# nanoporetech/medaka

Measured on NVIDIA H100. Metric: pileup positions/sec (consensus inference), higher is better.
Workload: dtype f32

## Files before the change

### medaka_b200/csrc/gru_wg.cu

```cuda
#include "common.cuh"
#include "ptx.cuh"
#include "rec_common.cuh"

namespace mdk {

constexpr int RW_THREADS = 256;
constexpr int RW_ABLK = (H / 8) * 64 * 16;
constexpr int RW_XBLK = 2 * 64 * 16;

template <int NT, bool FUSE_X, int OUT>
struct RwCfg {
    static constexpr int N = NT * RT_N;
    static constexpr bool HL = NT == 1;
    static constexpr int ROWS = HL ? 2 * N : N;
    static constexpr int PLANES = HL ? 1 : 2;
    static constexpr int KG = ROWS * 16 + 16;
    static constexpr int HPLANE = (H / 8) * KG;
    static constexpr int XPLANE = 2 * KG;
    static constexpr int HLO = HL ? N * 16 : HPLANE;
    static constexpr int XLO = HL ? N * 16 : XPLANE;
    static constexpr int RED = (RW_THREADS / 32) * NCLS * N;
    static constexpr int wlo_off = 0;
    static constexpr int wxlo_off = wlo_off + 6 * RW_ABLK;
    static constexpr int h_off = wxlo_off + (FUSE_X ? 6 * RW_XBLK : 0);
// ... 331 lines not shown
    dim3 grid((unsigned)((tiles + NT - 1) / NT), NDIR);
    constexpr bool LOGITS = OUT == OUT_LOGITS;
    kern<<<grid, RW_THREADS, smem_bytes, s>>>(gi, xin, w_hh_tm, b_hn, LOGITS ? nullptr : out, B, T, lin_w,
                                              LOGITS ? static_cast<float *>(out) : nullptr);
    return cudaGetLastError();
}

template <int NT>
static cudaError_t launch_rec_nt(const float *gi, const RecX *xin, const __half *w_hh_tm, const float *b_hn, int out_kind,
                                 void *out, const float *lin_w, int64_t B, int64_t T, cudaStream_t s) {
    if (xin)
        return out_kind == OUT_TILES ? launch_rec<NT, true, OUT_TILES>(gi, *xin, w_hh_tm, b_hn, out, nullptr, B, T, s)
                                     : cudaErrorInvalidValue;
    const RecX none{nullptr, nullptr, nullptr, 0};
    switch (out_kind) {
    case OUT_TILES: return launch_rec<NT, false, OUT_TILES>(gi, none, w_hh_tm, b_hn, out, nullptr, B, T, s);
    case OUT_ROWS: return launch_rec<NT, false, OUT_ROWS>(gi, none, w_hh_tm, b_hn, out, nullptr, B, T, s);
    case OUT_LOGITS:
        return lin_w ? launch_rec<NT, false, OUT_LOGITS>(gi, none, w_hh_tm, b_hn, out, lin_w, B, T, s) : cudaErrorInvalidValue;
    }
    return cudaErrorInvalidValue;
}

cudaError_t launch_rec_tc(const float *gi, const RecX *xin, const __half *w_hh_tm, const float *b_hn, int tiles_per_cta,
                          int out_kind, void *out, const float *lin_w, int64_t B, int64_t T, cudaStream_t s) {
    if (B == 0 || T == 0) return cudaSuccess;
    switch (tiles_per_cta) {
    case 1: return launch_rec_nt<1>(gi, xin, w_hh_tm, b_hn, out_kind, out, lin_w, B, T, s);
    case 2: return launch_rec_nt<2>(gi, xin, w_hh_tm, b_hn, out_kind, out, lin_w, B, T, s);
    }
    return cudaErrorInvalidValue;
}

constexpr int GW_THREADS = 256;
constexpr int GW_QK = 8;
constexpr int GW_STAGE_PLANE = GW_QK * XT_ROWS * 16;
constexpr int GW_STAGE = 2 * GW_STAGE_PLANE;
constexpr int GW_NQ = XT_K / 8 / GW_QK;
constexpr int GW_X_OFF = XT_TILE_BYTES;
constexpr int GW_BAR_OFF = GW_X_OFF + 2 * GW_STAGE;
constexpr int GW_SMEM = GW_BAR_OFF + 16;

__global__ void __launch_bounds__(GW_THREADS, 1)
gemm_tc_kernel(const uint8_t *__restrict__ x_tiles, const __half *__restrict__ w_in_tm, const float *__restrict__ bias,
               float *__restrict__ gi, int64_t P, int64_t ntiles) {
    extern __shared__ __align__(128) uint8_t smem[];
    uint64_t *full = reinterpret_cast<uint64_t *>(smem + GW_BAR_OFF);
    const int tid = threadIdx.x, wg = tid >> 7, warp = (tid >> 5) & 3, lane = tid & 31;
    const int gq = lane >> 2, cq = lane & 3;
    const int blk = blockIdx.x;
    const uint32_t sbase = smem_u32(smem);
    for (int i = tid; i < 2 * H * (H2 / 8); i += GW_THREADS) {
        const int kg = i & 31, r = (i >> 5) & (H - 1), p = i >> 12;
        const uint4 v = reinterpret_cast<const uint4 *>(w_in_tm + (((size_t)blk * 2 + p) * H + r) * H2)[kg];
        *reinterpret_cast<uint4 *>(smem + p * XT_PLANE_BYTES + kg * (XT_ROWS * 16) + r * 16) = v;
    }
    if (tid == 0) {
        mbar_init(&full[0], 1);
        mbar_init(&full[1], 1);
        fence_mbar_init();
    }
    fence_proxy_async_smem();
    __syncthreads();
    const int64_t my_tiles = blockIdx.y < ntiles ? (ntiles - 1 - blockIdx.y) / gridDim.y + 1 : 0;
    const int64_t nst = my_tiles * GW_NQ;
    auto issue = [&](int64_t it) {
        const int64_t tile = blockIdx.y + (it / GW_NQ) * gridDim.y;
        const int q = (int)(it % GW_NQ), s = (int)(it & 1);
        const uint8_t *src = x_tiles + tile * (int64_t)XT_TILE_BYTES + q * GW_STAGE_PLANE;
        mbar_arrive_expect_tx(&full[s], GW_STAGE);
        bulk_g2s(smem + GW_X_OFF + s * GW_STAGE, src, GW_STAGE_PLANE, &full[s]);
        bulk_g2s(smem + GW_X_OFF + s * GW_STAGE + GW_STAGE_PLANE, src + XT_PLANE_BYTES, GW_STAGE_PLANE, &full[s]);
    };
    if (tid == 0) {
        if (nst > 0) issue(0);
        if (nst > 1) issue(1);
    }
    const float bj[2] = {bias[blk * H + wg * 64 + warp * 16 + gq], bias[blk * H + wg * 64 + warp * 16 + gq + 8]};
    float acc[64];
#pragma unroll 1
    for (int64_t it = 0; it < nst; ++it) {
        const int q = (int)(it % GW_NQ), s = (int)(it & 1);
        mbar_wait(&full[s], (uint32_t)((it >> 1) & 1));
        wg_fence();
#pragma unroll
        for (int prod = 0; prod < 3; ++prod) {
            const int pa = prod == 2, pb = prod == 1;
#pragma unroll
            for (int kk = 0; kk < GW_QK / 2; ++kk) {
                const uint64_t a = make_smem_desc(sbase + pa * XT_PLANE_BYTES + (q * GW_QK + 2 * kk) * (XT_ROWS * 16) + wg * 64 * 16,
                                                  XT_ROWS * 16, 128);
                const uint64_t b = make_smem_desc(sbase + GW_X_OFF + s * GW_STAGE + pb * GW_STAGE_PLANE + 2 * kk * (XT_ROWS * 16),
                                                  XT_ROWS * 16, 128);
                Wgmma<128>::ss(acc, a, b, (q | prod | kk) ? 1u : 0u);
            }
        }
        wg_commit();
        wg_wait_all();
        wg_hold(acc);
        __syncthreads();
        if (tid == 0 && it + 2 < nst) issue(it + 2);
        if (q == GW_NQ - 1) {
            const int64_t tile = blockIdx.y + (it / GW_NQ) * gridDim.y;
            const int64_t prem = P - tile * XT_ROWS;
#pragma unroll
            for (int k = 0; k < 64; k += 2) {
                const int c = 8 * (k >> 2) + 2 * cq, hb = (k >> 1) & 1;
                if (c >= prem) continue;
                const int j = wg * 64 + warp * 16 + gq + 8 * hb;
                float *o = gi + ((((tile * (XT_ROWS / WT) + (c >> 4)) * 6 + blk) * 4 + ((c & 15) >> 2)) * H + j) * 4 + (c & 3);
                __stcs(reinterpret_cast<float2 *>(o), make_float2(acc[k] + bj[hb], acc[k + 1] + bj[hb]));
            }
        }
    }
}

cudaError_t launch_gemm_tc(const void *x_tiles, const __half *w_in_tm, const float *bias, float *gi, int64_t P,
                           int sm_count, cudaStream_t s) {
    if (P == 0) return cudaSuccess;
    const int64_t ntiles = (P + XT_ROWS - 1) / XT_ROWS;
    cudaError_t ea = cudaFuncSetAttribute(gemm_tc_kernel, cudaFuncAttributeMaxDynamicSharedMemorySize, GW_SMEM);
    if (ea != cudaSuccess) return ea;
    int64_t ct = sm_count / 6;
    if (ct < 1) ct = 1;
    if (ct > ntiles) ct = ntiles;
    dim3 grid(6, (unsigned)ct);
    gemm_tc_kernel<<<grid, GW_THREADS, GW_SMEM, s>>>(reinterpret_cast<const uint8_t *>(x_tiles), w_in_tm, bias, gi, P, ntiles);
    return cudaGetLastError();
}

__global__ void __launch_bounds__(256, 1)
selftest_kernel(const float *__restrict__ A, const float *__restrict__ Bm, float *__restrict__ D, int N, int K) {
    extern __shared__ __align__(128) uint8_t smem[];
    const int a_plane = 128 * K * 2, b_plane = N * K * 2;
    uint8_t *sa = smem, *sb = smem + 2 * a_plane;
    const int tid = threadIdx.x, wg = tid >> 7, warp = (tid >> 5) & 3, lane = tid & 31;
    for (int i = tid; i < 128 * K; i += 256) {
        const int r = i / K, k = i % K;
        __half hi, lo;
        split_f16(A[i], hi, lo);
        const int off = (k / 8) * (128 * 16) + r * 16 + (k % 8) * 2;
        *reinterpret_cast<__half *>(sa + off) = hi;
        *reinterpret_cast<__half *>(sa + a_plane + off) = lo;
    }
    for (int i = tid; i < N * K; i += 256) {
        const int r = i / K, k = i % K;
        __half hi, lo;
        split_f16(Bm[i], hi, lo);
        const int off = (k / 8) * (N * 16) + r * 16 + (k % 8) * 2;
        *reinterpret_cast<__half *>(sb + off) = hi;
        *reinterpret_cast<__half *>(sb + b_plane + off) = lo;
    }
    fence_proxy_async_smem();
    __syncthreads();
    for (int n0 = 0; n0 < N; n0 += 16) {
        float d[8];
        wg_fence();
        uint32_t acc = 0;
        for (int prod = 0; prod < 3; ++prod) {
            const int pa = (prod == 2), pb = (prod == 1);
// ... 40 lines not shown
```

### medaka_b200/csrc/ptx.cuh

```cuda
#pragma once
#include <cstdint>
#include <cuda_fp16.h>

namespace mdk {

__device__ __forceinline__ uint32_t smem_u32(const void *p) {
    return static_cast<uint32_t>(__cvta_generic_to_shared(p));
}

__device__ __forceinline__ void mbar_init(uint64_t *bar, uint32_t count) {
    asm volatile("mbarrier.init.shared::cta.b64 [%0], %1;" ::"r"(smem_u32(bar)), "r"(count) : "memory");
}
__device__ __forceinline__ void fence_mbar_init() {
    asm volatile("fence.mbarrier_init.release.cluster;" ::: "memory");
}
__device__ __forceinline__ void mbar_arrive_expect_tx(uint64_t *bar, uint32_t bytes) {
    asm volatile("mbarrier.arrive.expect_tx.shared::cta.b64 _, [%0], %1;" ::"r"(smem_u32(bar)), "r"(bytes)
                 : "memory");
}
__device__ __forceinline__ bool mbar_try_wait(uint64_t *bar, uint32_t parity) {
    uint32_t ok;
    asm volatile(
        "{\n\t.reg .pred p;\n\t"
        "mbarrier.try_wait.parity.shared::cta.b64 p, [%1], %2;\n\t"
        "selp.u32 %0, 1, 0, p;\n\t}"
        : "=r"(ok)
        : "r"(smem_u32(bar)), "r"(parity)
        : "memory");
    return ok != 0;
}
__device__ __forceinline__ void mbar_wait(uint64_t *bar, uint32_t parity) {
    if (mbar_try_wait(bar, parity)) return;
    const long long t0 = clock64();
    while (!mbar_try_wait(bar, parity)) {
        if (clock64() - t0 > 4000000000LL) __trap();
    }
}

__device__ __forceinline__ void fence_proxy_async_smem() {
    asm volatile("fence.proxy.async.shared::cta;" ::: "memory");
}

__device__ __forceinline__ uint32_t cluster_ctarank() {
    uint32_t r;
    asm volatile("mov.u32 %0, %%cluster_ctarank;" : "=r"(r));
    return r;
}
__device__ __forceinline__ uint32_t mapa_shared(uint32_t smem_addr, uint32_t rank) {
    uint32_t r;
    asm volatile("mapa.shared::cluster.u32 %0, %1, %2;" : "=r"(r) : "r"(smem_addr), "r"(rank));
    return r;
// ... 1 lines not shown
__device__ __forceinline__ void st_cluster_u32(uint32_t cluster_addr, uint32_t v) {
    asm volatile("st.shared::cluster.u32 [%0], %1;" ::"r"(cluster_addr), "r"(v) : "memory");
}
__device__ __forceinline__ void fence_proxy_async_cluster() {
    asm volatile("fence.proxy.async.shared::cluster;" ::: "memory");
}
__device__ __forceinline__ void mbar_arrive_cluster(uint32_t cluster_addr) {
    asm volatile("mbarrier.arrive.release.cluster.shared::cluster.b64 _, [%0];" ::"r"(cluster_addr) : "memory");
}
__device__ __forceinline__ bool mbar_try_wait_cluster(uint64_t *bar, uint32_t parity) {
    uint32_t ok;
    asm volatile(
        "{\n\t.reg .pred p;\n\t"
        "mbarrier.try_wait.parity.acquire.cluster.shared::cta.b64 p, [%1], %2;\n\t"
        "selp.u32 %0, 1, 0, p;\n\t}"
        : "=r"(ok)
        : "r"(smem_u32(bar)), "r"(parity)
        : "memory");
    return ok != 0;
}
__device__ __forceinline__ void mbar_wait_cluster(uint64_t *bar, uint32_t parity) {
    if (mbar_try_wait_cluster(bar, parity)) return;
    const long long t0 = clock64();
    while (!mbar_try_wait_cluster(bar, parity)) {
        if (clock64() - t0 > 4000000000LL) __trap();
    }
}
__device__ __forceinline__ void cluster_sync_all() {
    asm volatile("barrier.cluster.arrive.release.aligned;\n\tbarrier.cluster.wait.acquire.aligned;" ::: "memory");
}
__device__ __forceinline__ void named_bar_sync(uint32_t id, uint32_t count) {
    asm volatile("bar.sync %0, %1;" ::"r"(id), "r"(count) : "memory");
}

__device__ __forceinline__ void bulk_prefetch_l2(const void *gmem_src, uint32_t bytes) {
    asm volatile("cp.async.bulk.prefetch.L2.global [%0], %1;" ::"l"(gmem_src), "r"(bytes) : "memory");
}

__device__ __forceinline__ void bulk_g2s(void *smem_dst, const void *gmem_src, uint32_t bytes, uint64_t *bar) {
    asm volatile(
        "cp.async.bulk.shared::cluster.global.mbarrier::complete_tx::bytes [%0], [%1], %2, [%3];" ::"r"(
            smem_u32(smem_dst)),
        "l"(gmem_src), "r"(bytes), "r"(smem_u32(bar))
        : "memory");
}

__device__ __forceinline__ uint64_t make_smem_desc(uint32_t smem_addr, uint32_t lbo_bytes, uint32_t sbo_bytes) {
    uint64_t d = 0;
    d |= static_cast<uint64_t>((smem_addr & 0x3FFFF) >> 4);
    d |= static_cast<uint64_t>((lbo_bytes >> 4) & 0x3FFF) << 16;
    d |= static_cast<uint64_t>((sbo_bytes >> 4) & 0x3FFF) << 32;
    return d;
}
__device__ __forceinline__ void wg_fence() { asm volatile("wgmma.fence.sync.aligned;" ::: "memory"); }
__device__ __forceinline__ void wg_commit() { asm volatile("wgmma.commit_group.sync.aligned;" ::: "memory"); }
__device__ __forceinline__ void wg_wait_all() { asm volatile("wgmma.wait_group.sync.aligned 0;" ::: "memory"); }
template <int R>
__device__ __forceinline__ void wg_hold(float (&d)[R]) {
#pragma unroll
    for (int i = 0; i < R; ++i) asm volatile("" : "+f"(d[i])::"memory");
}

template <int N> struct Wgmma;
template <> struct Wgmma<16> {
    __device__ __forceinline__ static void ss(float (&d)[8], uint64_t a, uint64_t b, uint32_t accumulate) {
        asm volatile(
            "{\n\t.reg .pred p;\n\tsetp.ne.b32 p, %10, 0;\n\t"
            "wgmma.mma_async.sync.aligned.m64n16k16.f32.f16.f16 {%0,%1,%2,%3,%4,%5,%6,%7}, %8, %9, p, 1, 1, 0, 0;\n\t}"
            : "+f"(d[0]), "+f"(d[1]), "+f"(d[2]), "+f"(d[3]), "+f"(d[4]), "+f"(d[5]), "+f"(d[6]), "+f"(d[7])
            : "l"(a), "l"(b), "r"(accumulate));
    }
    __device__ __forceinline__ static void rs(float (&d)[8], const uint32_t (&a)[4], uint64_t b, uint32_t accumulate) {
        asm volatile(
            "{\n\t.reg .pred p;\n\tsetp.ne.b32 p, %13, 0;\n\t"
            "wgmma.mma_async.sync.aligned.m64n16k16.f32.f16.f16 {%0,%1,%2,%3,%4,%5,%6,%7}, {%8,%9,%10,%11}, %12, p, 1, 1, 0;\n\t}"
            : "+f"(d[0]), "+f"(d[1]), "+f"(d[2]), "+f"(d[3]), "+f"(d[4]), "+f"(d[5]), "+f"(d[6]), "+f"(d[7])
            : "r"(a[0]), "r"(a[1]), "r"(a[2]), "r"(a[3]), "l"(b), "r"(accumulate));
    }
    __device__ __forceinline__ static void ss(float (&d)[16], uint64_t a, uint64_t b, uint32_t accumulate) {
        asm volatile(
            "{\n\t.reg .pred p;\n\tsetp.ne.b32 p, %10, 0;\n\t"
            "wgmma.mma_async.sync.aligned.m64n16k16.f32.f16.f16 {%0,%1,%2,%3,%4,%5,%6,%7}, %8, %9, p, 1, 1, 0, 0;\n\t}"
            : "+f"(d[0]), "+f"(d[1]), "+f"(d[2]), "+f"(d[3]), "+f"(d[4]), "+f"(d[5]), "+f"(d[6]), "+f"(d[7])
            : "l"(a), "l"(b), "r"(accumulate));
    }
};
template <> struct Wgmma<32> {
    __device__ __forceinline__ static void ss(float (&d)[16], uint64_t a, uint64_t b, uint32_t accumulate) {
        asm volatile(
// ... 53 lines not shown
```

### medaka_b200/csrc/api.cu

```cuda
#include <algorithm>
#include <cstdlib>
#include <cstring>
#include <new>

#include "common.cuh"

namespace mdk {

static thread_local std::string g_last_error;

void set_error(const std::string &msg) { g_last_error = msg; }

int cuda_fail(cudaError_t err, const char *what, const char *file, int line) {
    char buf[512];
    snprintf(buf, sizeof(buf), "CUDA error %d (%s) at %s:%d: %s", (int)err, cudaGetErrorString(err), file, line, what);
    g_last_error = buf;
    if (err == cudaErrorMemoryAllocation) {
        cudaGetLastError();
        return MDK_ERR_NOMEM;
    }
    return MDK_ERR_CUDA;
}

template <typename T>
// ... 560 lines not shown
    }
    return MDK_OK;
}

int mdk_engine_timer_start(mdk_engine *e) {
    MDK_REQUIRE(e, MDK_ERR_ARG, "engine is NULL");
    MDK_CUDA(cudaSetDevice(e->device));
    int rc = mdk_engine_sync(e);
    if (rc) return rc;
    MDK_CUDA(cudaEventRecord(e->ev_timer[0], e->stream));
    for (int i = 1; i < mdk_engine::N_WS; ++i) MDK_CUDA(cudaStreamWaitEvent(e->ws[i].stream, e->ev_timer[0], 0));
    MDK_CUDA(cudaStreamWaitEvent(e->copy_in, e->ev_timer[0], 0));
    return MDK_OK;
}
int mdk_engine_timer_stop(mdk_engine *e, float *elapsed_ms) {
    MDK_REQUIRE(e && elapsed_ms, MDK_ERR_ARG, "NULL argument");
    MDK_CUDA(cudaSetDevice(e->device));
    int rc = launch_group(e);
    if (rc) return rc;
    for (int i = 1; i < mdk_engine::N_WS; ++i) {
        MDK_CUDA(cudaEventRecord(e->ev_join, e->ws[i].stream));
        MDK_CUDA(cudaStreamWaitEvent(e->stream, e->ev_join, 0));
    }
    MDK_CUDA(cudaEventRecord(e->ev_join, e->copy_out.stream));
    MDK_CUDA(cudaStreamWaitEvent(e->stream, e->ev_join, 0));
    MDK_CUDA(cudaEventRecord(e->ev_timer[1], e->stream));
    MDK_CUDA(cudaEventSynchronize(e->ev_timer[1]));
    MDK_CUDA(cudaEventElapsedTime(elapsed_ms, e->ev_timer[0], e->ev_timer[1]));
    return MDK_OK;
}

int mdk_engine_read_activation(mdk_engine *e, int which, float *out_host, int64_t n_floats) {
    MDK_REQUIRE(e && out_host, MDK_ERR_ARG, "NULL argument");
    MDK_REQUIRE(which == 0 || which == 1, MDK_ERR_ARG, "read_activation: which must be 0 or 1");
    mdk_ws &ln = e->ws[e->last_ws];
    const int64_t P = ln.last_B * ln.last_T;
    MDK_REQUIRE(P > 0 && n_floats == P * H2, MDK_ERR_ARG, "read_activation: size must be B*T*256 of the last forward");
    MDK_REQUIRE(!(which == 1 && ln.last_fused_head), MDK_ERR_STATE,
                "read_activation(1): the last forward fused the head into layer 1 (h1 never reached HBM); call "
                "mdk_engine_keep_activations(e, 1) before the forward");
    MDK_CUDA(cudaSetDevice(e->device));
    MDK_CUDA(cudaStreamSynchronize(ln.stream));
    if (ln.last_precision == MDK_PREC_FP32) {
        MDK_CUDA(cudaMemcpy(out_host, which == 1 ? (const void *)ln.h1 : (const void *)ln.h0,
                            (size_t)n_floats * sizeof(float), cudaMemcpyDeviceToHost));
    } else {
        float *tmp = nullptr;
        MDK_CUDA(cudaMalloc(&tmp, (size_t)n_floats * sizeof(float)));
        cudaError_t err = which == 0 ? launch_unpack_h0(ln.h0, tmp, ln.last_B, ln.last_T, ln.stream)
                                     : launch_untile_rows(ln.h1, tmp, ln.last_B, ln.last_T, ln.stream);
        if (err == cudaSuccess) err = cudaStreamSynchronize(ln.stream);
        if (err == cudaSuccess) err = cudaMemcpy(out_host, tmp, (size_t)n_floats * sizeof(float), cudaMemcpyDeviceToHost);
        cudaFree(tmp);
        e->launches++;
        if (err != cudaSuccess) return cuda_fail(err, "read_activation", __FILE__, __LINE__);
    }
    return MDK_OK;
}


int mdk_debug_read_plog(mdk_engine *e, float *out_host, int64_t n_floats) {
    MDK_REQUIRE(e && out_host, MDK_ERR_ARG, "NULL argument");
    mdk_ws &ln = e->ws[e->last_ws];
    MDK_REQUIRE(ln.last_fused_head, MDK_ERR_STATE, "read_plog: the last forward did not run the fused head");
    const int64_t tiles = (ln.last_B + WT - 1) / WT;
    MDK_REQUIRE(n_floats == NDIR * tiles * ln.last_T * PLOG_TS_FLOATS, MDK_ERR_ARG, "read_plog: size must be 2*tiles*T*80");
    MDK_CUDA(cudaSetDevice(e->device));
    MDK_CUDA(cudaStreamSynchronize(ln.stream));
    MDK_CUDA(cudaMemcpy(out_host, ln.plog, (size_t)n_floats * sizeof(float), cudaMemcpyDeviceToHost));
    return MDK_OK;
}

int64_t mdk_engine_launch_count(mdk_engine *e) { return e ? e->launches : 0; }

int mdk_engine_keep_activations(mdk_engine *e, int keep) {
    MDK_REQUIRE(e, MDK_ERR_ARG, "NULL engine");
    e->keep_act = keep != 0;
    return MDK_OK;
}

int64_t mdk_engine_preferred_windows(mdk_engine *e) {
    const int sms = e ? e->sm_count : 132;
    return (int64_t)mdk::WT * (sms / mdk::NDIR);
// ... 231 lines not shown
```

### medaka_b200/csrc/common.cuh

```cuda
#pragma once
#include <cuda_runtime.h>
#include <cuda_fp16.h>

#include <cstdint>
#include <cstdio>
#include <string>

#include "../../include/medaka_b200.h"
#include "packing.h"

namespace mdk {

constexpr int H = 128;
constexpr int G3 = 3 * H;
constexpr int NDIR = 2;
constexpr int GI_COLS = NDIR * G3;
constexpr int H2 = NDIR * H;
constexpr int NCLS = 5;

void set_error(const std::string &msg);
int cuda_fail(cudaError_t err, const char *what, const char *file, int line);

#define MDK_CUDA(call)                                                        \
    do {                                                                      \
// ... 137 lines not shown
    static constexpr int EV_RING = 32;
    cudaEvent_t evr[EV_RING][8] = {};
    cudaEvent_t *ev = evr[0];
    int64_t fwd_count = 0;
    cudaEvent_t ev_timer[2] = {};
    cudaEvent_t ev_join = nullptr;
    mdk::LayerWeights layer[2];
    float *lin_w = nullptr, *lin_b = nullptr;
    bool lin_loaded = false;
    bool keep_act = false;
    bool prepared = false;
    cudaStream_t copy_in = nullptr;
    mdk::CopyOut copy_out;
    mdk_timings last{};
    int64_t launches = 0;
};

namespace mdk {

cudaError_t launch_inproj0(const float *feats, const float *w_packed, const float *bias, float *gi,
                           int64_t P, int F, int64_t T, int tiled, cudaStream_t s);
cudaError_t launch_head(const float *h1, const float *lin_w, const float *lin_b, int64_t B, int64_t T, int tiled,
                        float *probs, float *logits, uint8_t *labels, cudaStream_t s);
cudaError_t launch_untile_rows(const float *src_tiled, float *dst, int64_t B, int64_t T, cudaStream_t s);
cudaError_t launch_normalise(const uint64_t *counts, const int64_t *major, const int64_t *minor, int64_t n,
                             int num_dtypes, int mode, int sym_indels, float *feats, int64_t *depth,
                             cudaStream_t s);
cudaError_t launch_decode(const float *probs, int64_t n, uint8_t *labels, uint8_t *quals, cudaStream_t s);
cudaError_t launch_decode_f64(const double *probs, int64_t n, uint8_t *labels, uint8_t *quals, cudaStream_t s);
cudaError_t launch_variant_columns(const int64_t *minor, const uint8_t *ref, const uint8_t *pred, int64_t n,
                                   uint8_t *out, cudaStream_t s);
cudaError_t launch_prepare_layer(const LayerWeights &lw, int in_features, bool build_in_tc, cudaStream_t s);
cudaError_t launch_unpack_h0(const void *h0_tiles, float *out, int64_t B, int64_t T, cudaStream_t s);
cudaError_t launch_rec_fp32(const float *gi, const float *w_hh_t, const float *b_hn, float *h_out, int64_t B,
                            int64_t T, cudaStream_t s);
cudaError_t launch_gemm_fp32(const float *A, const float *W, const float *bias, float *C, int64_t M, int K, int N,
                             cudaStream_t s);
struct RecX {
    const float *feats;
    const __half *w_x;
    const float *bias;
    int F;
};
enum { OUT_TILES = 0, OUT_ROWS = 1, OUT_LOGITS = 2 };
cudaError_t launch_rec_tc(const float *gi, const RecX *xin, const __half *w_hh_tm, const float *b_hn, int tiles_per_cta,
                          int out_kind, void *out, const float *lin_w, int64_t B, int64_t T, cudaStream_t s);
cudaError_t launch_head_plog(const float *plog, const float *lin_b, int64_t B, int64_t T, float *probs, float *logits,
                             uint8_t *labels, cudaStream_t s);
constexpr int PLOG_TS_FLOATS = NCLS * WT;
cudaError_t launch_gemm_tc(const void *x_tiles, const __half *w_in_tm, const float *bias, float *gi, int64_t P,
                           int sm_count, cudaStream_t s);
int selftest_umma(int device, const float *A, const float *B, float *D, int N, int K, int variant);
cudaError_t plp_scratch(size_t bytes, uint8_t **out, int slot);
int pileup_counts_dev(int64_t n_rec, const int32_t *pos, const uint16_t *flag, const uint8_t *mapq,
                      const uint8_t *dtype, const uint32_t *cigar, const int64_t *cigar_off, int64_t n_ops,
                      const uint8_t *seq, const int64_t *seq_off, int32_t start, int32_t end, int num_dtypes,
                      int min_mapq, int64_t max_cols, uint64_t *counts, int64_t *major, int64_t *minor,
                      int64_t *n_cols_host, cudaStream_t s);

}
```

### medaka_b200/csrc/misc.cu

```cuda
#include "common.cuh"
#include "ptx.cuh"

namespace mdk {

__device__ __forceinline__ bool feat_is_rev(int f10) { return f10 < 4 || f10 == 8; }

__device__ __forceinline__ int64_t lower_bound_major(const int64_t *__restrict__ major, int64_t n, int64_t key) {
    int64_t lo = 0, hi = n;
    while (lo < hi) {
        int64_t mid = (lo + hi) >> 1;
        if (major[mid] < key) lo = mid + 1; else hi = mid;
    }
    return lo;
}

template <int ND>
__global__ void __launch_bounds__(256) normalise_kernel(const uint64_t *__restrict__ counts,
                                                        const int64_t *__restrict__ major,
                                                        const int64_t *__restrict__ minor, int64_t n, int mode,
                                                        int sym_indels, float *__restrict__ feats,
                                                        int64_t *__restrict__ depth_out) {
    constexpr int F = 10 * ND;
    const int64_t i = blockIdx.x * (int64_t)blockDim.x + threadIdx.x;
    if (i >= n) return;
// ... 481 lines not shown
    }
    if (labels) labels[p] = (uint8_t)arg;
}

cudaError_t launch_head_plog(const float *plog, const float *lin_b, int64_t B, int64_t T, float *probs, float *logits,
                             uint8_t *labels, cudaStream_t s) {
    if (B == 0 || T == 0) return cudaSuccess;
    const int64_t tiles = (B + WT - 1) / WT;
    dim3 grid((unsigned)((T * WT + 255) / 256), (unsigned)tiles);
    head_plog_kernel<<<grid, 256, 0, s>>>(plog, lin_b, B, T, tiles * T, probs, logits, labels);
    return cudaGetLastError();
}

__global__ void unpack_h0_kernel(const __half *__restrict__ tiles, float *__restrict__ out, int64_t B, int64_t T) {
    const int64_t i = blockIdx.x * (int64_t)blockDim.x + threadIdx.x;
    if (i >= B * T * H2) return;
    const int64_t p = i / H2;
    const int k = (int)(i % H2);
    const int64_t row = tiled_row(p / T, p % T, T);
    const int64_t tile = row / XT_ROWS;
    const int r = (int)(row % XT_ROWS);
    const __half *base = tiles + tile * (XT_TILE_BYTES / 2);
    const int64_t off = (int64_t)(k / 8) * (XT_ROWS * 8) + r * 8 + (k % 8);
    out[i] = __half2float(base[off]) + __half2float(base[XT_PLANE_BYTES / 2 + off]);
}

cudaError_t launch_unpack_h0(const void *h0_tiles, float *out, int64_t B, int64_t T, cudaStream_t s) {
    const int64_t n = B * T * H2;
    if (n == 0) return cudaSuccess;
    unpack_h0_kernel<<<(unsigned)((n + 255) / 256), 256, 0, s>>>(reinterpret_cast<const __half *>(h0_tiles), out, B, T);
    return cudaGetLastError();
}

__global__ void untile_rows_kernel(const float *__restrict__ src, float *__restrict__ dst, int64_t B, int64_t T) {
    const int64_t i = blockIdx.x * (int64_t)blockDim.x + threadIdx.x;
    if (i >= B * T * H2) return;
    const int64_t p = i / H2;
    dst[i] = src[tiled_row(p / T, p % T, T) * H2 + (i % H2)];
}

cudaError_t launch_untile_rows(const float *src_tiled, float *dst, int64_t B, int64_t T, cudaStream_t s) {
    const int64_t n = B * T * H2;
    if (n == 0) return cudaSuccess;
    untile_rows_kernel<<<(unsigned)((n + 255) / 256), 256, 0, s>>>(src_tiled, dst, B, T);
    return cudaGetLastError();
}

}
```

### medaka_b200/models.py

```python
import collections
import inspect
import logging
import warnings

import numpy as np

from medaka_b200 import libmedaka as _lm

ForwardOutput = collections.namedtuple("ForwardOutput", ["probs", "logits", "labels"])

_PRECISIONS = {"tc": 0, "half": 0, "fp32": 1, "full": 1}


def _as_f32(x):
    if hasattr(x, "detach"):
        x = x.detach().cpu().numpy()
    return np.ascontiguousarray(x, dtype=np.float32)


class PinnedArray(object):

    def __init__(self, shape, dtype):
        lib = _lm.load()
        self.shape = tuple(int(s) for s in shape)
# ... 220 lines not shown

    def flush(self):
        _lm.check(_lm.lib.mdk_engine_flush(self._engine))

    def set_rec_mode(self, mode):
        code = {"auto": _lm.lib.MDK_REC_AUTO, "one": _lm.lib.MDK_REC_ONE_TILE, "pp": _lm.lib.MDK_REC_PINGPONG}[mode]
        _lm.check(_lm.lib.mdk_engine_set_rec_mode(self._engine, code))

    def set_group_windows(self, windows):
        _lm.check(_lm.lib.mdk_engine_set_group_windows(self._engine, int(windows)))

    def forward(self, x):
        import torch
        out = self.forward_arrays(_as_f32(x), want_logits=not self.normalise, want_labels=False)
        return torch.from_numpy(out.probs if self.normalise else out.logits)

    def predict_on_batch(self, batch):
        import torch
        out = self.forward_arrays(_as_f32(self.get_model_input_features(batch)), want_logits=False,
                                  want_labels=True)
        self.last_labels = out.labels
        return torch.from_numpy(out.probs)

    def last_timings(self):
        t = _lm.ffi.new("mdk_timings *")
        _lm.check(_lm.lib.mdk_engine_last_timings(self._engine, t))
        return {k: getattr(t, k) for k in ("h2d_ms", "inproj0_ms", "rec0_ms", "inproj1_ms", "rec1_ms",
                                             "head_ms", "d2h_ms", "total_ms", "launches")}

    def read_activation(self, which):
        t = self.last_timings()
        del t
        shape = self._last_shape
        out = np.empty((shape[0], shape[1], 2 * self.gru_size), dtype=np.float32)
        _lm.check(_lm.lib.mdk_engine_read_activation(
            self._engine, which, _lm.ffi.cast("float *", _lm.ffi.from_buffer(out)), out.size))
        return out

    def launch_count(self):
        return int(_lm.lib.mdk_engine_launch_count(self._engine))

    def keep_activations(self, keep=True):
        _lm.check(_lm.lib.mdk_engine_keep_activations(self._engine, 1 if keep else 0))

    def preferred_batch_size(self):
        return int(_lm.lib.mdk_engine_preferred_windows(self._engine))

    @property
    def engine(self):
        return self._engine

    def close(self):
        if self._engine is not None and _lm.lib is not None:
            _lm.lib.mdk_engine_destroy(self._engine)
            self._engine = None
        for p in self._pinned.values():
            p.close()
        self._pinned = {}

    def __del__(self):
        try:
            self.close()
        except Exception:
            pass


def model_from_dict(d, time_steps=None, device=0):
# ... 14 lines not shown
```

Before: 118.5 million.

## Warp-specialize input projection GEMM with TMA producer and ping-pong consumer warpgroups

Restructures the input-projection GEMM kernel. A dedicated producer warp now issues bulk copies into a 3-stage ring guarded by full/empty mbarriers. The two consumer warpgroups each handle whole tiles (both 64-row halves, 128 accumulators) in alternating ping-pong order, coordinated by named barriers. This lets one warpgroup's epilogue stores overlap the other's wgmma and removes the CTA-wide __syncthreads per stage. The cost is doubled accumulator register pressure, more shared memory for the ring, and more complex synchronisation.

```diff
diff --git a/medaka_b200/csrc/gru_wg.cu b/medaka_b200/csrc/gru_wg.cu
--- a/medaka_b200/csrc/gru_wg.cu
+++ b/medaka_b200/csrc/gru_wg.cu
@@ -387,22 +387,23 @@
     return cudaErrorInvalidValue;
 }
 
-constexpr int GW_THREADS = 256;
+constexpr int GW_THREADS = 288;
+constexpr int GW_RING = 3;
 constexpr int GW_QK = 8;
 constexpr int GW_STAGE_PLANE = GW_QK * XT_ROWS * 16;
 constexpr int GW_STAGE = 2 * GW_STAGE_PLANE;
 constexpr int GW_NQ = XT_K / 8 / GW_QK;
 constexpr int GW_X_OFF = XT_TILE_BYTES;
-constexpr int GW_BAR_OFF = GW_X_OFF + 2 * GW_STAGE;
-constexpr int GW_SMEM = GW_BAR_OFF + 16;
+constexpr int GW_BAR_OFF = GW_X_OFF + GW_RING * GW_STAGE;
+constexpr int GW_SMEM = GW_BAR_OFF + 2 * GW_RING * 8;
+static_assert(GW_SMEM <= 227 * 1024, "projection ring exceeds the shared memory of a CTA");
 
 __global__ void __launch_bounds__(GW_THREADS, 1)
 gemm_tc_kernel(const uint8_t *__restrict__ x_tiles, const __half *__restrict__ w_in_tm, const float *__restrict__ bias,
                float *__restrict__ gi, int64_t P, int64_t ntiles) {
     extern __shared__ __align__(128) uint8_t smem[];
-    uint64_t *full = reinterpret_cast<uint64_t *>(smem + GW_BAR_OFF);
+    uint64_t *full = reinterpret_cast<uint64_t *>(smem + GW_BAR_OFF), *empty = full + GW_RING;
     const int tid = threadIdx.x, wg = tid >> 7, warp = (tid >> 5) & 3, lane = tid & 31;
-    const int gq = lane >> 2, cq = lane & 3;
     const int blk = blockIdx.x;
     const uint32_t sbase = smem_u32(smem);
     for (int i = tid; i < 2 * H * (H2 / 8); i += GW_THREADS) {
@@ -411,60 +412,89 @@
         *reinterpret_cast<uint4 *>(smem + p * XT_PLANE_BYTES + kg * (XT_ROWS * 16) + r * 16) = v;
     }
     if (tid == 0) {
-        mbar_init(&full[0], 1);
-        mbar_init(&full[1], 1);
+        for (int s = 0; s < GW_RING; ++s) {
+            mbar_init(&full[s], 1);
+            mbar_init(&empty[s], 128);
+        }
         fence_mbar_init();
     }
     fence_proxy_async_smem();
     __syncthreads();
     const int64_t my_tiles = blockIdx.y < ntiles ? (ntiles - 1 - blockIdx.y) / gridDim.y + 1 : 0;
-    const int64_t nst = my_tiles * GW_NQ;
-    auto issue = [&](int64_t it) {
-        const int64_t tile = blockIdx.y + (it / GW_NQ) * gridDim.y;
-        const int q = (int)(it % GW_NQ), s = (int)(it & 1);
-        const uint8_t *src = x_tiles + tile * (int64_t)XT_TILE_BYTES + q * GW_STAGE_PLANE;
-        mbar_arrive_expect_tx(&full[s], GW_STAGE);
-        bulk_g2s(smem + GW_X_OFF + s * GW_STAGE, src, GW_STAGE_PLANE, &full[s]);
-        bulk_g2s(smem + GW_X_OFF + s * GW_STAGE + GW_STAGE_PLANE, src + XT_PLANE_BYTES, GW_STAGE_PLANE, &full[s]);
-    };
-    if (tid == 0) {
-        if (nst > 0) issue(0);
-        if (nst > 1) issue(1);
-    }
-    const float bj[2] = {bias[blk * H + wg * 64 + warp * 16 + gq], bias[blk * H + wg * 64 + warp * 16 + gq + 8]};
-    float acc[64];
+
+    if (wg == 2) {
+        if (lane == 0) {
+            const int64_t nst = my_tiles * GW_NQ;
 #pragma unroll 1
-    for (int64_t it = 0; it < nst; ++it) {
-        const int q = (int)(it % GW_NQ), s = (int)(it & 1);
-        mbar_wait(&full[s], (uint32_t)((it >> 1) & 1));
-        wg_fence();
-#pragma unroll
-        for (int prod = 0; prod < 3; ++prod) {
-            const int pa = prod == 2, pb = prod == 1;
-#pragma unroll
-            for (int kk = 0; kk < GW_QK / 2; ++kk) {
-                const uint64_t a = make_smem_desc(sbase + pa * XT_PLANE_BYTES + (q * GW_QK + 2 * kk) * (XT_ROWS * 16) + wg * 64 * 16,
-                                                  XT_ROWS * 16, 128);
-                const uint64_t b = make_smem_desc(sbase + GW_X_OFF + s * GW_STAGE + pb * GW_STAGE_PLANE + 2 * kk * (XT_ROWS * 16),
-                                                  XT_ROWS * 16, 128);
-                Wgmma<128>::ss(acc, a, b, (q | prod | kk) ? 1u : 0u);
-            }
-        }
-        wg_commit();
-        wg_wait_all();
-        wg_hold(acc);
-        __syncthreads();
-        if (tid == 0 && it + 2 < nst) issue(it + 2);
-        if (q == GW_NQ - 1) {
-            const int64_t tile = blockIdx.y + (it / GW_NQ) * gridDim.y;
-            const int64_t prem = P - tile * XT_ROWS;
+            for (int64_t it = 0; it < nst; ++it) {
+                const int64_t tile = blockIdx.y + (it / GW_NQ) * gridDim.y;
+                const int q = (int)(it % GW_NQ), s = (int)(it % GW_RING);
+                const int64_t pass = it / GW_RING;
+                if (pass > 0) mbar_wait(&empty[s], (uint32_t)((pass - 1) & 1));
+                const uint8_t *src = x_tiles + tile * (int64_t)XT_TILE_BYTES + q * GW_STAGE_PLANE;
+                mbar_arrive_expect_tx(&full[s], GW_STAGE);
+                bulk_g2s(smem + GW_X_OFF + s * GW_STAGE, src, GW_STAGE_PLANE, &full[s]);
+                bulk_g2s(smem + GW_X_OFF + s * GW_STAGE + GW_STAGE_PLANE, src + XT_PLANE_BYTES, GW_STAGE_PLANE, &full[s]);
+            }
+        }
+        return;
+    }
+
+    const int gq = lane >> 2, cq = lane & 3;
+    float bj[2][2];
+#pragma unroll
+    for (int half = 0; half < 2; ++half) {
+        bj[half][0] = bias[blk * H + half * 64 + warp * 16 + gq];
+        bj[half][1] = bias[blk * H + half * 64 + warp * 16 + gq + 8];
+    }
+    float acc[2][64];
+#pragma unroll 1
+    for (int64_t n = wg; n < my_tiles; n += 2) {
+        if (n > 0) named_bar_sync(1 + wg, 2 * 128);
+        const int64_t it0 = n * GW_NQ;
+#pragma unroll
+        for (int q = 0; q < GW_NQ; ++q) {
+            const int s = (int)((it0 + q) % GW_RING);
+            mbar_wait(&full[s], (uint32_t)(((it0 + q) / GW_RING) & 1));
+            wg_fence();
+#pragma unroll
+            for (int prod = 0; prod < 3; ++prod) {
+                const int pa = prod == 2, pb = prod == 1;
+#pragma unroll
+                for (int kk = 0; kk < GW_QK / 2; ++kk) {
+                    const uint64_t b = make_smem_desc(sbase + GW_X_OFF + s * GW_STAGE + pb * GW_STAGE_PLANE + 2 * kk * (XT_ROWS * 16),
+                                                      XT_ROWS * 16, 128);
+#pragma unroll
+                    for (int half = 0; half < 2; ++half) {
+                        const uint64_t a = make_smem_desc(sbase + pa * XT_PLANE_BYTES + (q * GW_QK + 2 * kk) * (XT_ROWS * 16) +
+                                                              half * 64 * 16,
+                                                          XT_ROWS * 16, 128);
+                        Wgmma<128>::ss(acc[half], a, b, (q | prod | kk) ? 1u : 0u);
+                    }
+                }
+            }
+            wg_commit();
+            if (q == GW_NQ - 1 && n + 1 < my_tiles) named_bar_arrive(2 - wg, 2 * 128);
+            if (q > 0) {
+                wg_wait<1>();
+                mbar_arrive(&empty[(it0 + q - 1) % GW_RING]);
+            }
+        }
+        wg_wait<0>();
+        wg_hold(acc[0]);
+        wg_hold(acc[1]);
+        mbar_arrive(&empty[(it0 + GW_NQ - 1) % GW_RING]);
+        const int64_t tile = blockIdx.y + n * gridDim.y;
+        const int64_t prem = P - tile * XT_ROWS;
+#pragma unroll
+        for (int half = 0; half < 2; ++half) {
 #pragma unroll
             for (int k = 0; k < 64; k += 2) {
                 const int c = 8 * (k >> 2) + 2 * cq, hb = (k >> 1) & 1;
                 if (c >= prem) continue;
-                const int j = wg * 64 + warp * 16 + gq + 8 * hb;
+                const int j = half * 64 + warp * 16 + gq + 8 * hb;
                 float *o = gi + ((((tile * (XT_ROWS / WT) + (c >> 4)) * 6 + blk) * 4 + ((c & 15) >> 2)) * H + j) * 4 + (c & 3);
-                __stcs(reinterpret_cast<float2 *>(o), make_float2(acc[k] + bj[hb], acc[k + 1] + bj[hb]));
+                __stcs(reinterpret_cast<float2 *>(o), make_float2(acc[half][k] + bj[half][hb], acc[half][k + 1] + bj[half][hb]));
             }
         }
     }
diff --git a/medaka_b200/csrc/ptx.cuh b/medaka_b200/csrc/ptx.cuh
--- a/medaka_b200/csrc/ptx.cuh
+++ b/medaka_b200/csrc/ptx.cuh
@@ -13,6 +13,9 @@
 }
 __device__ __forceinline__ void fence_mbar_init() {
     asm volatile("fence.mbarrier_init.release.cluster;" ::: "memory");
+}
+__device__ __forceinline__ void mbar_arrive(uint64_t *bar) {
+    asm volatile("mbarrier.arrive.shared::cta.b64 _, [%0];" ::"r"(smem_u32(bar)) : "memory");
 }
 __device__ __forceinline__ void mbar_arrive_expect_tx(uint64_t *bar, uint32_t bytes) {
     asm volatile("mbarrier.arrive.expect_tx.shared::cta.b64 _, [%0], %1;" ::"r"(smem_u32(bar)), "r"(bytes)
@@ -84,6 +87,9 @@
 __device__ __forceinline__ void named_bar_sync(uint32_t id, uint32_t count) {
     asm volatile("bar.sync %0, %1;" ::"r"(id), "r"(count) : "memory");
 }
+__device__ __forceinline__ void named_bar_arrive(uint32_t id, uint32_t count) {
+    asm volatile("bar.arrive %0, %1;" ::"r"(id), "r"(count) : "memory");
+}
 
 __device__ __forceinline__ void bulk_prefetch_l2(const void *gmem_src, uint32_t bytes) {
     asm volatile("cp.async.bulk.prefetch.L2.global [%0], %1;" ::"l"(gmem_src), "r"(bytes) : "memory");
@@ -107,6 +113,8 @@
 __device__ __forceinline__ void wg_fence() { asm volatile("wgmma.fence.sync.aligned;" ::: "memory"); }
 __device__ __forceinline__ void wg_commit() { asm volatile("wgmma.commit_group.sync.aligned;" ::: "memory"); }
 __device__ __forceinline__ void wg_wait_all() { asm volatile("wgmma.wait_group.sync.aligned 0;" ::: "memory"); }
+template <int N>
+__device__ __forceinline__ void wg_wait() { asm volatile("wgmma.wait_group.sync.aligned %0;" ::"n"(N) : "memory"); }
 template <int R>
 __device__ __forceinline__ void wg_hold(float (&d)[R]) {
 #pragma unroll
```

Measured after the change: 119.1 million (median of 6 runs). No clear change (+0.5%).

## Pipeline the tensor-core input projection with a 3-stage ring and overlapped epilogue

Applied to the files above, without the earlier changes.

The input-projection GEMM kernel moves from a 2-slot double buffer guarded by a full __syncthreads to a 3-slot ring with per-stage full/empty mbarriers. Only the first warp waits for a slot to drain before refilling it. The kernel keeps one wgmma group in flight, alternates two accumulator sets, and interleaves each tile's output stores with the next tile's MMAs, which is meant to hide load latency and epilogue time. It also drops the tail-row bound check, relying on padded tiles. A debug readback path for the projected gates is added, and the higher register and shared-memory use could lower occupancy or cause spills.

```diff
diff --git a/medaka_b200/csrc/api.cu b/medaka_b200/csrc/api.cu
--- a/medaka_b200/csrc/api.cu
+++ b/medaka_b200/csrc/api.cu
@@ -616,13 +616,17 @@
 
 int mdk_engine_read_activation(mdk_engine *e, int which, float *out_host, int64_t n_floats) {
     MDK_REQUIRE(e && out_host, MDK_ERR_ARG, "NULL argument");
-    MDK_REQUIRE(which == 0 || which == 1, MDK_ERR_ARG, "read_activation: which must be 0 or 1");
+    MDK_REQUIRE(which >= 0 && which <= 2, MDK_ERR_ARG, "read_activation: which must be 0, 1 or 2");
     mdk_ws &ln = e->ws[e->last_ws];
     const int64_t P = ln.last_B * ln.last_T;
-    MDK_REQUIRE(P > 0 && n_floats == P * H2, MDK_ERR_ARG, "read_activation: size must be B*T*256 of the last forward");
+    const int64_t width = which == 2 ? GI_COLS : H2;
+    MDK_REQUIRE(P > 0 && n_floats == P * width, MDK_ERR_ARG,
+                "read_activation: size must be B*T*256 (B*T*768 for which = 2) of the last forward");
     MDK_REQUIRE(!(which == 1 && ln.last_fused_head), MDK_ERR_STATE,
                 "read_activation(1): the last forward fused the head into layer 1 (h1 never reached HBM); call "
                 "mdk_engine_keep_activations(e, 1) before the forward");
+    MDK_REQUIRE(!(which == 2 && ln.last_precision != MDK_PREC_TC), MDK_ERR_STATE,
+                "read_activation(2): the last forward did not run the tensor-core projection");
     MDK_CUDA(cudaSetDevice(e->device));
     MDK_CUDA(cudaStreamSynchronize(ln.stream));
     if (ln.last_precision == MDK_PREC_FP32) {
@@ -631,8 +635,9 @@
     } else {
         float *tmp = nullptr;
         MDK_CUDA(cudaMalloc(&tmp, (size_t)n_floats * sizeof(float)));
-        cudaError_t err = which == 0 ? launch_unpack_h0(ln.h0, tmp, ln.last_B, ln.last_T, ln.stream)
-                                     : launch_untile_rows(ln.h1, tmp, ln.last_B, ln.last_T, ln.stream);
+        cudaError_t err = which == 0   ? launch_unpack_h0(ln.h0, tmp, ln.last_B, ln.last_T, ln.stream)
+                          : which == 1 ? launch_untile_rows(ln.h1, tmp, ln.last_B, ln.last_T, ln.stream)
+                                       : launch_unpack_gi(ln.gi, tmp, ln.last_B, ln.last_T, ln.stream);
         if (err == cudaSuccess) err = cudaStreamSynchronize(ln.stream);
         if (err == cudaSuccess) err = cudaMemcpy(out_host, tmp, (size_t)n_floats * sizeof(float), cudaMemcpyDeviceToHost);
         cudaFree(tmp);
diff --git a/medaka_b200/csrc/common.cuh b/medaka_b200/csrc/common.cuh
--- a/medaka_b200/csrc/common.cuh
+++ b/medaka_b200/csrc/common.cuh
@@ -193,6 +193,7 @@
                                    uint8_t *out, cudaStream_t s);
 cudaError_t launch_prepare_layer(const LayerWeights &lw, int in_features, bool build_in_tc, cudaStream_t s);
 cudaError_t launch_unpack_h0(const void *h0_tiles, float *out, int64_t B, int64_t T, cudaStream_t s);
+cudaError_t launch_unpack_gi(const float *gi, float *out, int64_t B, int64_t T, cudaStream_t s);
 cudaError_t launch_rec_fp32(const float *gi, const float *w_hh_t, const float *b_hn, float *h_out, int64_t B,
                             int64_t T, cudaStream_t s);
 cudaError_t launch_gemm_fp32(const float *A, const float *W, const float *bias, float *C, int64_t M, int K, int N,
diff --git a/medaka_b200/csrc/gru_wg.cu b/medaka_b200/csrc/gru_wg.cu
--- a/medaka_b200/csrc/gru_wg.cu
+++ b/medaka_b200/csrc/gru_wg.cu
@@ -392,15 +392,18 @@
 constexpr int GW_STAGE_PLANE = GW_QK * XT_ROWS * 16;
 constexpr int GW_STAGE = 2 * GW_STAGE_PLANE;
 constexpr int GW_NQ = XT_K / 8 / GW_QK;
+constexpr int GW_RING = 3;
 constexpr int GW_X_OFF = XT_TILE_BYTES;
-constexpr int GW_BAR_OFF = GW_X_OFF + 2 * GW_STAGE;
-constexpr int GW_SMEM = GW_BAR_OFF + 16;
+constexpr int GW_BAR_OFF = GW_X_OFF + GW_RING * GW_STAGE;
+constexpr int GW_SMEM = GW_BAR_OFF + 2 * GW_RING * 8;
+static_assert(GW_SMEM <= 227 * 1024, "smem budget");
 
 __global__ void __launch_bounds__(GW_THREADS, 1)
 gemm_tc_kernel(const uint8_t *__restrict__ x_tiles, const __half *__restrict__ w_in_tm, const float *__restrict__ bias,
-               float *__restrict__ gi, int64_t P, int64_t ntiles) {
+               float *__restrict__ gi, int64_t ntiles) {
     extern __shared__ __align__(128) uint8_t smem[];
     uint64_t *full = reinterpret_cast<uint64_t *>(smem + GW_BAR_OFF);
+    uint64_t *empty = full + GW_RING;
     const int tid = threadIdx.x, wg = tid >> 7, warp = (tid >> 5) & 3, lane = tid & 31;
     const int gq = lane >> 2, cq = lane & 3;
     const int blk = blockIdx.x;
@@ -411,8 +414,10 @@
         *reinterpret_cast<uint4 *>(smem + p * XT_PLANE_BYTES + kg * (XT_ROWS * 16) + r * 16) = v;
     }
     if (tid == 0) {
-        mbar_init(&full[0], 1);
-        mbar_init(&full[1], 1);
+        for (int s = 0; s < GW_RING; ++s) {
+            mbar_init(&full[s], 1);
+            mbar_init(&empty[s], 2);
+        }
         fence_mbar_init();
     }
     fence_proxy_async_smem();
@@ -421,22 +426,23 @@
     const int64_t nst = my_tiles * GW_NQ;
     auto issue = [&](int64_t it) {
         const int64_t tile = blockIdx.y + (it / GW_NQ) * gridDim.y;
-        const int q = (int)(it % GW_NQ), s = (int)(it & 1);
+        const int q = (int)(it % GW_NQ), s = (int)(it % GW_RING);
         const uint8_t *src = x_tiles + tile * (int64_t)XT_TILE_BYTES + q * GW_STAGE_PLANE;
         mbar_arrive_expect_tx(&full[s], GW_STAGE);
         bulk_g2s(smem + GW_X_OFF + s * GW_STAGE, src, GW_STAGE_PLANE, &full[s]);
         bulk_g2s(smem + GW_X_OFF + s * GW_STAGE + GW_STAGE_PLANE, src + XT_PLANE_BYTES, GW_STAGE_PLANE, &full[s]);
     };
-    if (tid == 0) {
-        if (nst > 0) issue(0);
-        if (nst > 1) issue(1);
-    }
-    const float bj[2] = {bias[blk * H + wg * 64 + warp * 16 + gq], bias[blk * H + wg * 64 + warp * 16 + gq + 8]};
-    float acc[64];
-#pragma unroll 1
-    for (int64_t it = 0; it < nst; ++it) {
-        const int q = (int)(it % GW_NQ), s = (int)(it & 1);
-        mbar_wait(&full[s], (uint32_t)((it >> 1) & 1));
+    if (tid == 0)
+        for (int64_t it = 0; it < GW_RING && it < nst; ++it) issue(it);
+
+    const int jr = wg * 64 + warp * 16 + gq;
+    const float bj[2] = {bias[blk * H + jr], bias[blk * H + jr + 8]};
+    float acc0[64], acc1[64];
+    int64_t it = 0;
+    const bool warp0 = __shfl_sync(0xffffffffu, tid < 32, 0);
+    auto stage = [&](float (&acc)[64], int q) {
+        const int s = (int)(it % GW_RING);
+        mbar_wait(&full[s], (uint32_t)((it / GW_RING) & 1));
         wg_fence();
 #pragma unroll
         for (int prod = 0; prod < 3; ++prod) {
@@ -451,22 +457,54 @@
             }
         }
         wg_commit();
-        wg_wait_all();
+        wg_wait<1>();
+        if (it > 0) {
+            const int sp = (int)((it - 1) % GW_RING);
+            if ((tid & 127) == 0) mbar_arrive(&empty[sp]);
+            if (warp0 && it + 2 < nst) {
+                mbar_wait(&empty[sp], (uint32_t)(((it - 1) / GW_RING) & 1));
+                if (lane == 0) issue(it + 2);
+            }
+        }
+        ++it;
+    };
+    float *const gthr = gi + ((int64_t)blk * 4 + (cq >> 1)) * (H * 4) + jr * 4 + 2 * (cq & 1);
+    auto epilogue = [&](float (&acc)[64], int64_t lt, int part) {
         wg_hold(acc);
-        __syncthreads();
-        if (tid == 0 && it + 2 < nst) issue(it + 2);
-        if (q == GW_NQ - 1) {
-            const int64_t tile = blockIdx.y + (it / GW_NQ) * gridDim.y;
-            const int64_t prem = P - tile * XT_ROWS;
-#pragma unroll
-            for (int k = 0; k < 64; k += 2) {
-                const int c = 8 * (k >> 2) + 2 * cq, hb = (k >> 1) & 1;
-                if (c >= prem) continue;
-                const int j = wg * 64 + warp * 16 + gq + 8 * hb;
-                float *o = gi + ((((tile * (XT_ROWS / WT) + (c >> 4)) * 6 + blk) * 4 + ((c & 15) >> 2)) * H + j) * 4 + (c & 3);
-                __stcs(reinterpret_cast<float2 *>(o), make_float2(acc[k] + bj[hb], acc[k + 1] + bj[hb]));
-            }
-        }
+        float *const o = gthr + (blockIdx.y + lt * gridDim.y) * (int64_t)(XT_ROWS / WT) * GI_TS_FLOATS;
+#pragma unroll
+        for (int k = 16 * part; k < 16 * part + 16; k += 2) {
+            const int i = k >> 2, hb = (k >> 1) & 1;
+            __stcs(reinterpret_cast<float2 *>(o + (i >> 1) * GI_TS_FLOATS + (2 * (i & 1) * H + 8 * hb) * 4),
+                   make_float2(acc[k] + bj[hb], acc[k + 1] + bj[hb]));
+        }
+    };
+    int64_t lt = 0;
+#pragma unroll 1
+    for (; lt + 1 < my_tiles; lt += 2) {
+#pragma unroll
+        for (int q = 0; q < GW_NQ; ++q) {
+            stage(acc0, q);
+            if (lt > 0) epilogue(acc1, lt - 1, q);
+        }
+#pragma unroll
+        for (int q = 0; q < GW_NQ; ++q) {
+            stage(acc1, q);
+            epilogue(acc0, lt, q);
+        }
+    }
+    if (lt < my_tiles) {
+#pragma unroll
+        for (int q = 0; q < GW_NQ; ++q) {
+            stage(acc0, q);
+            if (lt > 0) epilogue(acc1, lt - 1, q);
+        }
+    }
+    wg_wait_all();
+#pragma unroll
+    for (int q = 0; q < GW_NQ; ++q) {
+        if (lt < my_tiles) epilogue(acc0, lt, q);
+        else if (lt > 0) epilogue(acc1, lt - 1, q);
     }
 }
 
@@ -480,7 +518,7 @@
     if (ct < 1) ct = 1;
     if (ct > ntiles) ct = ntiles;
     dim3 grid(6, (unsigned)ct);
-    gemm_tc_kernel<<<grid, GW_THREADS, GW_SMEM, s>>>(reinterpret_cast<const uint8_t *>(x_tiles), w_in_tm, bias, gi, P, ntiles);
+    gemm_tc_kernel<<<grid, GW_THREADS, GW_SMEM, s>>>(reinterpret_cast<const uint8_t *>(x_tiles), w_in_tm, bias, gi, ntiles);
     return cudaGetLastError();
 }
 
diff --git a/medaka_b200/csrc/misc.cu b/medaka_b200/csrc/misc.cu
--- a/medaka_b200/csrc/misc.cu
+++ b/medaka_b200/csrc/misc.cu
@@ -537,6 +537,20 @@
     return cudaGetLastError();
 }
 
+__global__ void unpack_gi_kernel(const float *__restrict__ gi, float *__restrict__ out, int64_t B, int64_t T) {
+    const int64_t i = blockIdx.x * (int64_t)blockDim.x + threadIdx.x;
+    if (i >= B * T * GI_COLS) return;
+    const int64_t p = i / GI_COLS;
+    out[i] = gi[gi_quad_index(tiled_row(p / T, p % T, T), (int)(i % GI_COLS))];
+}
+
+cudaError_t launch_unpack_gi(const float *gi, float *out, int64_t B, int64_t T, cudaStream_t s) {
+    const int64_t n = B * T * GI_COLS;
+    if (n == 0) return cudaSuccess;
+    unpack_gi_kernel<<<(unsigned)((n + 255) / 256), 256, 0, s>>>(gi, out, B, T);
+    return cudaGetLastError();
+}
+
 __global__ void untile_rows_kernel(const float *__restrict__ src, float *__restrict__ dst, int64_t B, int64_t T) {
     const int64_t i = blockIdx.x * (int64_t)blockDim.x + threadIdx.x;
     if (i >= B * T * H2) return;
diff --git a/medaka_b200/csrc/ptx.cuh b/medaka_b200/csrc/ptx.cuh
--- a/medaka_b200/csrc/ptx.cuh
+++ b/medaka_b200/csrc/ptx.cuh
@@ -17,6 +17,9 @@
 __device__ __forceinline__ void mbar_arrive_expect_tx(uint64_t *bar, uint32_t bytes) {
     asm volatile("mbarrier.arrive.expect_tx.shared::cta.b64 _, [%0], %1;" ::"r"(smem_u32(bar)), "r"(bytes)
                  : "memory");
+}
+__device__ __forceinline__ void mbar_arrive(uint64_t *bar) {
+    asm volatile("mbarrier.arrive.shared::cta.b64 _, [%0];" ::"r"(smem_u32(bar)) : "memory");
 }
 __device__ __forceinline__ bool mbar_try_wait(uint64_t *bar, uint32_t parity) {
     uint32_t ok;
@@ -107,6 +110,8 @@
 __device__ __forceinline__ void wg_fence() { asm volatile("wgmma.fence.sync.aligned;" ::: "memory"); }
 __device__ __forceinline__ void wg_commit() { asm volatile("wgmma.commit_group.sync.aligned;" ::: "memory"); }
 __device__ __forceinline__ void wg_wait_all() { asm volatile("wgmma.wait_group.sync.aligned 0;" ::: "memory"); }
+template <int N>
+__device__ __forceinline__ void wg_wait() { asm volatile("wgmma.wait_group.sync.aligned %0;" ::"n"(N) : "memory"); }
 template <int R>
 __device__ __forceinline__ void wg_hold(float (&d)[R]) {
 #pragma unroll
diff --git a/medaka_b200/models.py b/medaka_b200/models.py
--- a/medaka_b200/models.py
+++ b/medaka_b200/models.py
@@ -276,7 +276,8 @@
         t = self.last_timings()
         del t
         shape = self._last_shape
-        out = np.empty((shape[0], shape[1], 2 * self.gru_size), dtype=np.float32)
+        width = 6 * self.gru_size if which == 2 else 2 * self.gru_size
+        out = np.empty((shape[0], shape[1], width), dtype=np.float32)
         _lm.check(_lm.lib.mdk_engine_read_activation(
             self._engine, which, _lm.ffi.cast("float *", _lm.ffi.from_buffer(out)), out.size))
         return out
```

After: 116.9 million before, 121.4 million after (median of 6 runs). +3.8%, better.
